# MustaphaMensouri/Distributed-Continuous-Training-with-Airflow-PyTorch-Distributed-DDP-

Measured on AMD Instinct MI355X. Metric: samples/sec (whole node) for weather-MLP DDP, higher is better.
Workload: dtype fp32; 1 GPU; global_batch=4, per_rank_batch=4, parallelism=dp1, optimizer=adam lr=0.01, loss=ce, engine=fused-persistent, dataset_rows=8649, features=5

## Files before the change

### distributed-continuous-training-with-airflow-pytorch-distributed-ddp-_amd/csrc/knobs.cpp

```cpp
#include "knobs.h"

#include <cstdlib>
#include <cstring>

namespace dct {

namespace {
Knobs g_knobs;
bool g_loaded = false;

int env_int(const char* name, int dflt) {
  const char* e = std::getenv(name);
  return (e && *e) ? std::atoi(e) : dflt;
}
}

void knobs_reload() {
  Knobs k;
  const char* mk = std::getenv("DCT_MLP_KERNEL");
  k.mlp_force_lds = (mk && std::strcmp(mk, "lds") == 0) ? 1 : 0;
  if (const char* b = std::getenv("DCT_MLP_BLOCK")) k.mlp_block = (b[0] == '0') ? 0 : (b[0] == '3' ? 3 : (b[0] == '8' ? 8 : -1));
  k.fused_head = env_int("DCT_FUSED_HEAD", 1) != 0;
  k.dw_into_adam = env_int("DCT_DW_INTO_ADAM", 1) != 0;
  k.reducer_inline = env_int("DCT_REDUCER_INLINE", -2);
  if (k.reducer_inline > 1 || k.reducer_inline < -2) k.reducer_inline = -2;
  k.rccl_one_rank = env_int("DCT_RCCL_ONE_RANK", 0) == 1;
  k.reducer_standin_us = env_int("DCT_REDUCER_STANDIN_US", 0);
  k.reducer_standin_wgs = env_int("DCT_REDUCER_STANDIN_WGS", 16);
  k.reducer_flag_edges = env_int("DCT_REDUCER_FLAG_EDGES", 1) != 0;
  if (k.reducer_standin_us < 0) k.reducer_standin_us = 0;
  if (k.reducer_standin_wgs < 1) k.reducer_standin_wgs = 1;
  if (k.reducer_standin_wgs > 1024) k.reducer_standin_wgs = 1024;
  g_knobs = k;
  g_loaded = true;
}

const Knobs& knobs() {
  if (!g_loaded) knobs_reload();
  return g_knobs;
}

}

extern "C" void dct_knobs_reload() { dct::knobs_reload(); }
```

### distributed-continuous-training-with-airflow-pytorch-distributed-ddp-_amd/csrc/knobs.h

```cpp
#pragma once

namespace dct {

struct Knobs {
  int mlp_force_lds = 0;
  int mlp_block = -1;
  int fused_head = 1;
  int dw_into_adam = 1;
  int reducer_inline = -2;
  int reducer_standin_us = 0;
  int reducer_standin_wgs = 16;
  int reducer_flag_edges = 1;
  int rccl_one_rank = 0;
};

const Knobs& knobs();
void knobs_reload();

}
```

### distributed-continuous-training-with-airflow-pytorch-distributed-ddp-_amd/csrc/mlp_block5.hip

```cpp
#include "mlp_block5_impl.h"

namespace dct {

void mlp_launch_block5_xg(int world, size_t bytes, hipStream_t st, const MlpShape& sh, const MlpArgs& a);
void mlp_launch_block5_b8(size_t bytes, hipStream_t st, const MlpShape& sh, const MlpArgs& a);

static bool b5_xg_world_ok(int w) { return w >= 2 && w <= 8; }

bool mlp_block5_ok(const MlpShape& sh, const MlpArgs& a) {
  const bool aligned = (sh.woff[1] % 4) == 0 && ((uintptr_t)a.p & 15) == 0 && (((uintptr_t)a.m | (uintptr_t)a.v) & 15) == 0;
  const bool xg_ok = a.xg_world <= 1 ||
                     (a.mode == 0 && b5_xg_world_ok(a.xg_world) && a.xg_rank >= 0 && a.xg_rank < a.xg_world &&
                      a.xg_recv != nullptr && a.xg_peers != nullptr && a.xg_status != nullptr &&
                      (a.prof == nullptr || a.xg_world == 2 || a.xg_world == 4 || a.xg_world == 8));
  const bool b8_ok = (a.B <= blk5::B && sh.mlp_block != 8) || a.prof == nullptr;
  return aligned && b8_ok && mlp_block5_shape_ok(sh.dims, sh.L, a.B) &&
         ((a.mode == 0 && a.cursor == nullptr) || (a.mode == 1 && a.steps == 1 && a.grad_out != nullptr)) &&
         (a.loss_kind == 0 || a.loss_kind == 1) && a.pending == nullptr && (a.stage == nullptr || a.mode == 1) && xg_ok;
}

bool mlp_block5_shape_ok(const int* dims, int L, int B) {
  return L == 3 && dims[1] == blk5::H && dims[2] == blk5::H && dims[0] >= 1 && dims[0] <= blk5::DMAX &&
         dims[3] == blk5::C && B >= 1 && B <= blk5::BMAX;
}

size_t mlp_block5_xg_bytes(int world) {
  switch (world) {
    case 2: return (size_t)b5x::Lay<2>::BYTES;
    case 4: return (size_t)b5x::Lay<4>::BYTES;
    case 8: return (size_t)b5x::Lay<8>::BYTES;
    case 3: return (size_t)b5x::Lay<3>::BYTES;
    case 5: return (size_t)b5x::Lay<5>::BYTES;
    case 6: return (size_t)b5x::Lay<6>::BYTES;
    case 7: return (size_t)b5x::Lay<7>::BYTES;
    default: return 0;
  }
}

hipError_t mlp_launch_block5(const MlpShape& sh, const MlpArgs& a, hipStream_t st) {
  const size_t bytes = (size_t)blk5::LDS_FLOATS * sizeof(float);
  const bool wd = a.wd != 0.f;
  if (a.B > blk5::B || sh.mlp_block == 8) {
    mlp_launch_block5_b8(bytes, st, sh, a);
  } else if (a.xg_world > 1) {
    mlp_launch_block5_xg(a.xg_world, bytes, st, sh, a);
  } else if (a.mode == 1) {
    if (a.loss_kind == 0) b5_launch<false, 0, false, true, false>(bytes, st, sh, a);
    else b5_launch<false, 1, false, true, false>(bytes, st, sh, a);
  } else if (a.prof) {
    if (a.loss_kind == 0) b5_launch<true, 0, true>(bytes, st, sh, a);
    else b5_launch<true, 1, true>(bytes, st, sh, a);
  } else if (a.loss_kind == 0) {
    if (wd) b5_launch<true, 0>(bytes, st, sh, a);
    else b5_launch<false, 0>(bytes, st, sh, a);
  } else {
    if (wd) b5_launch<true, 1>(bytes, st, sh, a);
    else b5_launch<false, 1>(bytes, st, sh, a);
  }
  return hipGetLastError();
}

}
```

### distributed-continuous-training-with-airflow-pytorch-distributed-ddp-_amd/csrc/mlp_block5_impl.h

```cpp
#pragma once
#include <type_traits>

#include "mlp_block_util.h"

namespace dct {

namespace blk5 {
constexpr int H = 128, NT = 512, NW = 8, KS = 16, DMAX = 8, B = 4, C = 2, MBMAX = 2, BMAX = B * MBMAX;
constexpr int PSTR = 36;
template <int MB>
struct Lds {
  static constexpr int RB = B * MB;
  static constexpr int XT = 0;
  static constexpr int LAB = XT + 3 * DMAX * RB;
  static constexpr int MSK = LAB + (MB == 1 ? 16 : 32);
  static constexpr int LOGP = MSK + 2 * NW * 2;
  static constexpr int H1W = LOGP + 2 * NW * 8;
  static constexpr int H1X = H1W + MB * NW * KS * 4;
  static constexpr int PART = H1X + NW * KS * 4;
  static constexpr int W2L = PART + 2 * H * PSTR;
  static constexpr int B2L = W2L + 2 * H * C;
  static constexpr int ABT = B2L + 8;
  static constexpr int TOTAL = ABT + 4;
  static_assert((H1W % 4) == 0 && (PART % 4) == 0 && (MSK % 4) == 0 && (LAB % 4) == 0 && (W2L % 4) == 0 &&
                    (B2L % 4) == 0 && (H1X % 4) == 0 && (LOGP % 4) == 0,
                "16-B aligned tiles");
};
static_assert(Lds<1>::TOTAL == 11036, "the batch <= 4 layout is round 5's");
constexpr int STG = H * H;
constexpr int LDS_FLOATS = Lds<MBMAX>::TOTAL > 2 * STG ? Lds<MBMAX>::TOTAL : 2 * STG;
static_assert(LDS_FLOATS * 4 <= 160 * 1024, "fits the CU");
using Stg = bku::Stage<H, NT>;
constexpr float LOG2E = 1.4426950408889634f, LN2 = 0.6931471805599453f;
}

namespace b5x {
typedef unsigned int v4u __attribute__((ext_vector_type(4)));
constexpr int SYS = 17;
constexpr int NP = 16, NS = 2;
constexpr int G = blk5::NT * 16;
template <int XW>
struct Lay {
  static constexpr int NO = (NP + XW - 1) / XW;
  static constexpr int RSS = NO + NS;
  static constexpr int AG = 2 * XW * RSS * G;
  static constexpr int LS = AG + 2 * (NP + NS) * G;
  static constexpr int EP = LS + ((2 * XW * 16 + 255) & ~255);
  static constexpr int BYTES = EP + (NP + NS) * 2 * G;
  static __device__ __forceinline__ int rs(int par, int src, int slot) { return ((par * XW + src) * RSS + slot) * G; }
  static __device__ __forceinline__ int ag(int par, int slot) { return AG + (par * (NP + NS) + slot) * G; }
  static __device__ __forceinline__ int ls(int par, int src) { return LS + (par * XW + src) * 16; }
  static __device__ __forceinline__ int ep(int slot, int mv) { return EP + (slot * 2 + mv) * G; }
};
__device__ __forceinline__ void put(__amdgpu_buffer_rsrc_t rs, int off, float x, float y, uint32_t tag) {
  v4u d;
  d.x = __float_as_uint(x);
  d.y = tag;
  d.z = __float_as_uint(y);
  d.w = tag;
  __builtin_amdgcn_raw_buffer_store_b128(d, rs, off, 0, SYS);
}
__device__ __forceinline__ bool get(__amdgpu_buffer_rsrc_t rs, int off, uint32_t tag, float& x, float& y) {
  const v4u d = __builtin_amdgcn_raw_buffer_load_b128(rs, off, 0, SYS);
  x = __uint_as_float(d.x);
  y = __uint_as_float(d.z);
  return (d.y == tag) & (d.w == tag);
}
template <int XW, class T>
__device__ __forceinline__ T pick(const T* v, int rank) {
  T r = v[0];
#pragma unroll
  for (int k = 1; k < XW; ++k) r = rank == k ? v[k] : r;
  return r;
}
template <int V>
using IC = std::integral_constant<int, V>;
template <int N, int I = 0, class F>
__device__ __host__ __forceinline__ void static_for(F&& f) {
  if constexpr (I < N) {
    f(IC<I>{});
    static_for<N, I + 1>(f);
  }
}
}

#define B5STAMP(k)                                              \
  if constexpr (PROF) {                                         \
    const unsigned long long t_ = __builtin_amdgcn_s_memtime(); \
    pacc[(k)] += t_ - t_last;                                   \
    t_last = t_;                                                \
  }

__device__ __forceinline__ uint32_t b5_elem(int li, int r, int u) {
  return ((uint32_t)((li * 64 + r) * 65536 + u) + 0x165667B1u) * 0xC2B2AE3Du;
}
__device__ __forceinline__ float b5_drop(uint32_t seed, uint32_t gstep, uint32_t elem, float p, float scale) {
  uint32_t h = (seed * 0x9E3779B1u) ^ ((gstep + 0x7F4A7C15u) * 0x85EBCA77u);
  h ^= elem;
  h ^= h >> 16;
  h *= 0x7feb352du;
  h ^= h >> 15;
  h *= 0x846ca68bu;
  h ^= h >> 16;
  return u01(h) < p ? 0.f : scale;
}

template <bool WD>
__device__ __forceinline__ void adam_pair(float& p0, float g0, float& m0, float& v0, float& p1, float g1, float& m1,
                                          float& v1, float b1, float b2, float wd, float A, float E) {
  if constexpr (WD) { g0 = fmaf(wd, p0, g0); g1 = fmaf(wd, p1, g1); }
  m0 = fmaf(b1, m0, g0);
  m1 = fmaf(b1, m1, g1);
  v0 = fmaf(b2, v0, g0 * g0);
  v1 = fmaf(b2, v1, g1 * g1);
  const float d0 = fmaf(__builtin_amdgcn_sqrtf(v0), A, E), d1 = fmaf(__builtin_amdgcn_sqrtf(v1), A, E);
  const float R = __builtin_amdgcn_rcpf(d0 * d1);
  p0 = fmaf(-m0, d1 * R, p0);
  p1 = fmaf(-m1, d0 * R, p1);
}

__device__ __forceinline__ bku::f32x4_t quad_transpose_mf(const float (&v)[4], const float (&e)[4]) {
  bku::f32x4_t t = (bku::f32x4_t){0.f, 0.f, 0.f, 0.f};
#pragma unroll
  for (int i = 0; i < 4; ++i) t = bku::mfma4(v[i], e[i], t);
  return t;
}

__device__ __forceinline__ float rs_bits2to5(float (&P)[16], int lane) {
  using namespace bku;
#pragma unroll
  for (int i = 0; i < 8; ++i) P[i] = swap32_sum(P[i], P[i + 8]);
#pragma unroll
  for (int i = 0; i < 4; ++i) P[i] = swap16_sum(P[i], P[i + 4]);
  const bool b3 = (lane >> 3) & 1, b2 = (lane >> 2) & 1;
#pragma unroll
  for (int i = 0; i < 2; ++i) {
    const float keep = b3 ? P[i + 2] : P[i], send = b3 ? P[i] : P[i + 2];
    P[i] = keep + dpp<ROR8>(send);
  }
  const float keep = b2 ? P[1] : P[0], send = b2 ? P[0] : P[1];
  const float t4 = dpp<ROR4>(send), t12 = dpp<0x12C>(send);
  return keep + (b2 ? t4 : t12);
}

typedef float v2f __attribute__((ext_vector_type(2)));
template <bool WD>
__device__ __forceinline__ void adam_v2(v2f& p, v2f g, v2f& m, v2f& v, float b1, float b2, float wd, float A, float E) {
  if constexpr (WD) g = (v2f)(wd) * p + g;
  m = (v2f)(b1) * m + g;
  v = (v2f)(b2) * v + g * g;
  const v2f sq = (v2f){__builtin_amdgcn_sqrtf(v.x), __builtin_amdgcn_sqrtf(v.y)};
  const v2f d = sq * (v2f)(A) + (v2f)(E);
  const float R = __builtin_amdgcn_rcpf(d.x * d.y);
  p = p - m * ((v2f){d.y, d.x} * R);
}

template <bool WD, int LK, bool PROF = false, bool DXM = true, bool ADAM = true, int XW = 1, int RK = -1, int MB = 1>
__global__ __launch_bounds__(blk5::NT, 1) void mlp_block5_kernel(MlpShape sh, MlpArgs a) {
  using namespace blk5;
  using namespace bku;
  static_assert(XW == 1 || (ADAM && XW >= 2 && XW <= 8), "exchange: train mode, 2..8 ranks");
  static_assert(MB >= 1 && MB <= MBMAX, "micro-batches per step");
  using LY = Lds<MB>;
  constexpr int RB = LY::RB, XT = LY::XT, LAB = LY::LAB, MSK = LY::MSK, LOGP = LY::LOGP, H1W = LY::H1W;
  constexpr int H1X = LY::H1X, PART = LY::PART, W2L = LY::W2L, B2L = LY::B2L, ABT = LY::ABT, TOTAL = LY::TOTAL;
  constexpr int PS = XW > 1 ? 32 : 16;
  using XL = b5x::Lay<XW>;
  constexpr int NO = XL::NO;
  extern __shared__ __attribute__((aligned(16))) float lds[];
  const int tid = threadIdx.x, w = tid >> 6, l = tid & 63;
  const int D0 = sh.dims[0];
  const int r0 = l & 3;
  const int u = KS * w + (l >> 2);
  const int wo0 = sh.woff[0], bo0 = sh.boff[0], wo1 = sh.woff[1], bo1 = sh.boff[1];
  const int wo2 = sh.woff[2], bo2 = sh.boff[2];
  unsigned long long pacc[PROF ? PS : 1] = {};
  unsigned long long t_last = PROF ? __builtin_amdgcn_s_memtime() : 0ull;
  const unsigned long long t_kstart = t_last;

  const int Bsz = a.B;
  const int fb = tid & (RB - 1), fd = tid / RB;
  const int nel = Bsz * D0;
  int role = 0, pb = 0, pk = 0;
  if (tid < nel) { role = 1; pb = tid / D0; pk = tid - pb * D0; }
  else if (tid < nel + Bsz) { role = 2; pb = tid - nel; }
  const bool stp = !ADAM && a.stage != nullptr;
  uint32_t st_tag = 0u, st_x = 0u, st_lab = 0u;
  if (stp) {
    st_tag = a.stage[0];
    if (tid < RB * DMAX && fd < D0 && fb < Bsz) st_x = a.stage[64 + fb * D0 + fd];
    if (tid < Bsz) st_lab = a.stage[64 + nel + tid];
  }
  const int cur0 = (!ADAM && a.cursor) ? sload(a.cursor) : 0;
  const int bs0 = min(Bsz, a.n_items - cur0 * Bsz);
  const bool first_ok = tid < RB * DMAX && fb < bs0;
  const int rb_raw = a.idx[max(0, min(cur0 * Bsz + (first_ok ? fb : 0), a.n_items - 1))];
  const int rb_first = (first_ok && !stp) ? rb_raw : 0;
  int ridx_next = 0;
  if (!stp && role && (cur0 + 1) * Bsz + pb < a.n_items) ridx_next = a.idx[(cur0 + 1) * Bsz + pb];

  v4f sp[Stg::LD], sm[Stg::LD], sv[Stg::LD];
#pragma unroll
  for (int i = 0; i < Stg::LD; ++i) {
    const int f = wo1 + 4 * (i * NT + tid);
    sp[i] = *reinterpret_cast<const v4f*>(a.p + f);
    if constexpr (ADAM) sm[i] = *reinterpret_cast<const v4f*>(a.m + f);
  }
  if constexpr (ADAM) {
#pragma unroll
    for (int i = 0; i < Stg::LD; ++i) sv[i] = *reinterpret_cast<const v4f*>(a.v + wo1 + 4 * (i * NT + tid));
  }
  float w0[2], m0[2], v0[2];
#pragma unroll
  for (int i = 0; i < 2; ++i) {
    const int d = r0 + 4 * i;
    const bool ok = d < D0;
    const int f = wo0 + u * D0 + (ok ? d : 0);
    w0[i] = ok ? a.p[f] : 0.f;
    m0[i] = (ok && ADAM) ? a.m[f] : 0.f;
    v0[i] = (ok && ADAM) ? a.v[f] : 0.f;
  }
  float pb0 = a.p[bo0 + u], mb0 = ADAM ? a.m[bo0 + u] : 0.f, vb0 = ADAM ? a.v[bo0 + u] : 0.f;
  float pw2[C];
#pragma unroll
  for (int c = 0; c < C; ++c) pw2[c] = a.p[wo2 + c * H + u];
  const bool own_w2 = r0 < C;
  const int fw2 = wo2 + (XW > 1 ? (r0 & 1) : (own_w2 ? r0 : 0)) * H + u;
  float mw2 = ((own_w2 || XW > 1) && ADAM) ? a.m[fw2] : 0.f, vw2 = ((own_w2 || XW > 1) && ADAM) ? a.v[fw2] : 0.f;
  float pb1 = a.p[bo1 + u], mb1 = ADAM ? a.m[bo1 + u] : 0.f, vb1 = ADAM ? a.v[bo1 + u] : 0.f;
  const bool own_b2 = w == 0 && l < C;
  const int fb2 = bo2 + (own_b2 ? l : 0);
  float pb2 = own_b2 ? a.p[fb2] : 0.f, mb2 = (own_b2 && ADAM) ? a.m[fb2] : 0.f, vb2 = (own_b2 && ADAM) ? a.v[fb2] : 0.f;
  const int fbx = r0 == 0 ? bo0 + u : (r0 == 1 ? bo1 + u : bo2 + (l & 1));
  float pbx = 0.f, mbx = 0.f, vbx = 0.f;
  if constexpr (XW > 1) {
    pbx = a.p[fbx];
    mbx = a.m[fbx];
    vbx = a.v[fbx];
  }

  int t0 = a.t0;
  uint32_t step_base = a.step_base;
  if (a.step_counter) {
    t0 = sload(a.step_counter);
    step_base = (uint32_t)t0;
// ... 47 lines not shown
  const uint32_t* pf_base = role == 1 ? reinterpret_cast<const uint32_t*>(a.X) + pk : reinterpret_cast<const uint32_t*>(a.Y);
  const int pf_stride = role == 1 ? a.ldx : (role == 2 ? 1 : 0);
  lds_barrier();

  if constexpr (PROF) pacc[14] = __builtin_amdgcn_s_memtime() - t_kstart;
  const float p_drop = a.dropout;
  const bool drop = p_drop > 0.f;
  const float scale = XW > 1 ? a.k_drop_scale : (drop ? 1.0f / (1.0f - p_drop) : 1.0f);
  const float l2b1 = XW > 1 ? a.k_l2b1 : log2f(a.b1), l2b2 = XW > 1 ? a.k_l2b2 : log2f(a.b2);
  const float c1 = 1.f - a.b1, c2 = 1.f - a.b2;
  const float rc1 = XW > 1 ? a.k_rc1 : 1.f / c1, rc2 = XW > 1 ? a.k_rc2 : 1.f / c2;
  const float sqc2 = XW > 1 ? a.k_sqc2 : sqrtf(c2);
#pragma unroll
  for (int j = 0; j < 2; ++j)
#pragma unroll
    for (int k = 0; k < KS; ++k) { m1[j][k] *= rc1; v1[j][k] *= rc2; }
#pragma unroll
  for (int i = 0; i < 2; ++i) { m0[i] *= rc1; v0[i] *= rc2; }
  mb0 *= rc1; vb0 *= rc2; mw2 *= rc1; vw2 *= rc2; mb1 *= rc1; vb1 *= rc2; mb2 *= rc1; vb2 *= rc2;
  mbx *= rc1; vbx *= rc2;
  v2f W[2][KS / 2], Mo[2][KS / 2], Vo[2][KS / 2];
#pragma unroll
  for (int j = 0; j < 2; ++j)
#pragma unroll
    for (int h = 0; h < KS / 2; ++h) {
      W[j][h] = (v2f){w1[j][2 * h], w1[j][2 * h + 1]};
      Mo[j][h] = (v2f){m1[j][2 * h], m1[j][2 * h + 1]};
      Vo[j][h] = (v2f){v1[j][2 * h], v1[j][2 * h + 1]};
    }
  const int xrank = XW > 1 ? (RK >= 0 ? RK : a.xg_rank) : 0;
  v2f MoO[NO], VoO[NO];
  __amdgpu_buffer_rsrc_t xrr = __builtin_amdgcn_make_buffer_rsrc((void*)a.xg_recv, 0, 0, 0x00020000), xpr[XW];
  const bool sown = XW == 1 || (__builtin_amdgcn_readfirstlane(w) % XW) == xrank;
  bool xbad = false;
  unsigned long long xticks = 0;
  if constexpr (XW > 1) {
#pragma unroll
    for (int t = 0; t < NO; ++t) {
      v2f cm[XW], cv[XW];
#pragma unroll
      for (int k = 0; k < XW; ++k) {
        const int i = XW * t + k < b5x::NP ? XW * t + k : 0;
        cm[k] = Mo[i >> 3][i & 7];
        cv[k] = Vo[i >> 3][i & 7];
      }
      MoO[t] = b5x::pick<XW>(cm, xrank);
      VoO[t] = b5x::pick<XW>(cv, xrank);
    }
  }
  if constexpr (XW > 1) {
    xrr = __builtin_amdgcn_make_buffer_rsrc((void*)a.xg_recv, 0, XL::BYTES, 0x00020000);
#pragma unroll
    for (int q = 0; q < XW; ++q)
      xpr[q] = __builtin_amdgcn_make_buffer_rsrc((void*)sload_ptr(a.xg_peers, q), 0, XL::BYTES, 0x00020000);
  }
  auto xwait = [&](uint32_t tag, auto&& sweep) -> bool {
    const unsigned long long t_start = __builtin_amdgcn_s_memrealtime();
    for (int spin = 0;; ++spin) {
      asm volatile("" ::: "memory");
      if (__all(sweep())) return true;
      if ((spin & 15) == 15 && (long long)(__builtin_amdgcn_s_memrealtime() - t_start) > a.xg_timeout) {
        if (l == 0) __hip_atomic_store(a.xg_status, tag, __ATOMIC_RELAXED, __HIP_MEMORY_SCOPE_SYSTEM);
        return false;
      }
      __builtin_amdgcn_s_sleep(1);
    }
  };
  const int tb = tid * 16;
  uint32_t el0[MB], el1[MB];
  float f1[MB], f2[MB];
#pragma unroll
  for (int hf = 0; hf < MB; ++hf) {
    el0[hf] = b5_elem(0, r0 + B * hf, u);
    el1[hf] = b5_elem(1, r0 + B * hf, u);
    f1[hf] = b5_drop(a.seed, step_base, el0[hf], p_drop, scale);
    f2[hf] = b5_drop(a.seed, step_base, el1[hf], p_drop, scale);
  }
  float* h1x = lds + H1X + w * (KS * 4);
  float eye[4];
#pragma unroll
  for (int i = 0; i < 4; ++i) eye[i] = r0 == i ? 1.f : 0.f;
  const int cb = (l >> 2) & 1;
  int xb = 0;
  if (a.tune == 1 && w >= NW / 2) __builtin_amdgcn_s_setprio(1);
  if (a.tune == 2 && w < NW / 2) __builtin_amdgcn_s_setprio(1);
  if constexpr (PROF) {
    t_last = __builtin_amdgcn_s_memtime();
    pacc[9] = t_last - t_kstart;
  }
  for (int s = 0; s < a.steps; ++s) {
    const int sb = s + cur0;
    const int bs = min(Bsz, a.n_items - sb * Bsz);
    const uint32_t gstep = step_base + (uint32_t)s;
    const int xbn = xb == 2 ? 0 : xb + 1;
    const int pbuf = s & 1, nbuf = pbuf ^ 1;
    const float* xT = lds + XT + xb * DMAX * RB;
    const bool have_next = (s + 1 < a.steps);
    const int bs_next = have_next ? min(Bsz, a.n_items - (sb + 1) * Bsz) : 0;
    const uint32_t raw_next = pf_base[(size_t)ridx_next * pf_stride];
    const int nx2 = min((sb + 2) * Bsz + pb, a.n_items - 1);
    const int ridx_next2 = a.idx[nx2 < 0 ? 0 : nx2];
    const uint32_t xtag = gstep + 1u;
    const int xpar = (int)(gstep & 1u);
    const int t = t0 + s + 1;
    float dz2m[MB][2][4];
    float dz = 0.f, xbl = 0.f, tls = 0.f;
    float h2 = 0.f, h1 = 0.f;
    float gw0s = 0.f, gw1s = 0.f, gb1s = 0.f, gbs = 0.f, g0s = 0.f, g1s = 0.f, db0s = 0.f;
    float aA = 0.f, aE = 0.f;
    v2f GO[NO];
#pragma unroll
    for (int t2 = 0; t2 < NO; ++t2) GO[t2] = (v2f){0.f, 0.f};
    float xg_own = 0.f, xg_bx = 0.f;
    v2f xs_g0 = (v2f){0.f, 0.f}, xs_g1 = (v2f){0.f, 0.f};
    bool abort_step = false;
    auto dw1_pass = [&]() {
#pragma unroll
      for (int q = 0; q < KS / 4; ++q) {
        f32x4_t g[2];
#pragma unroll
        for (int j = 0; j < 2; ++j) g[j] = (f32x4_t){0.f, 0.f, 0.f, 0.f};
#pragma unroll
        for (int hf = 0; hf < MB; ++hf) {
          const float4 hq = *reinterpret_cast<const float4*>(lds + H1W + (hf * NW + w) * (KS * 4) + (4 * q + r0) * 4);
          const float hv[4] = {hq.x, hq.y, hq.z, hq.w};
#pragma unroll
          for (int j = 0; j < 2; ++j)
#pragma unroll
            for (int r = 0; r < 4; ++r) g[j] = mfma4(hv[r], dz2m[hf][j][r], g[j]);
        }

        if constexpr (ADAM && XW > 1) {
#pragma unroll
          for (int j = 0; j < 2; ++j)
#pragma unroll
            for (int h = 0; h < 2; ++h) {
              const int i = 8 * j + 2 * q + h;
              const float gx = g[j][2 * h], gy = g[j][2 * h + 1];
              if ((i % XW) == xrank) GO[i / XW] = (v2f){gx, gy};
              else b5x::put(xpr[i % XW], XL::rs(xpar, (xrank - i % XW + XW) % XW, i / XW) + tb, gx, gy, xtag);
            }
        } else if constexpr (ADAM) {
#pragma unroll
          for (int j = 0; j < 2; ++j)
#pragma unroll
            for (int h = 0; h < 2; ++h)
              adam_v2<WD>(W[j][2 * q + h], (v2f){g[j][2 * h], g[j][2 * h + 1]}, Mo[j][2 * q + h], Vo[j][2 * q + h], a.b1,
                          a.b2, a.wd, aA, aE);
        } else {
#pragma unroll
          for (int j = 0; j < 2; ++j)
            *reinterpret_cast<float4*>(a.grad_out + wo1 + (l + 64 * j) * H + KS * w + 4 * q) =
                make_float4(g[j][0], g[j][1], g[j][2], g[j][3]);
        }
      }
    };

#pragma unroll
    for (int hf = 0; hf < MB; ++hf) {
      const bool last = hf == MB - 1;
      const int mpar = MB == 1 ? pbuf : hf;
      float* h1w = lds + H1W + (hf * NW + w) * (KS * 4);

      const float4 xa = *reinterpret_cast<const float4*>(xT + r0 * RB + B * hf);
      const float4 xc = *reinterpret_cast<const float4*>(xT + (r0 + 4) * RB + B * hf);
      {
        const float acc0 = w0[0] * xa.x + w0[1] * xc.x, acc1 = w0[0] * xa.y + w0[1] * xc.y;
        const float acc2 = w0[0] * xa.z + w0[1] * xc.z, acc3 = w0[0] * xa.w + w0[1] * xc.w;
        const bool qb1 = (r0 >> 1) & 1, qb0 = r0 & 1;
        const float k0 = qb1 ? acc2 : acc0, k1 = qb1 ? acc3 : acc1;
        const float s0 = qb1 ? acc0 : acc2, s1 = qb1 ? acc1 : acc3;
        const float e0 = k0 + dpp<QP_X2>(s0), e1 = k1 + dpp<QP_X2>(s1);
        const float kq = qb0 ? e1 : e0, sq = qb0 ? e0 : e1;
        h1 = fmaxf(kq + dpp<QP_X1>(sq) + pb0, 0.f) * f1[hf];
        h1w[l] = h1;
        h1x[r0 * KS + (l >> 2)] = h1;
      }
      __builtin_amdgcn_wave_barrier();
      B5STAMP(0)
      {
        f32x4_t cq[2][KS / 4];
#pragma unroll
        for (int q = 0; q < KS / 4; ++q) {
          const float4 hq = *reinterpret_cast<const float4*>(h1x + r0 * KS + 4 * q);
          const float hv[4] = {hq.x, hq.y, hq.z, hq.w};
#pragma unroll
          for (int j = 0; j < 2; ++j) {
            cq[j][q] = (f32x4_t){0.f, 0.f, 0.f, 0.f};
#pragma unroll
            for (int e = 0; e < 4; ++e) cq[j][q] = mfma4(hv[e], W[j][2 * q + (e >> 1)][e & 1], cq[j][q]);
          }
        }
        f32x4_t cj[2];
#pragma unroll
        for (int j = 0; j < 2; ++j) cj[j] = (cq[j][0] + cq[j][1]) + (cq[j][2] + cq[j][3]);
        float* part = lds + PART + mpar * (H * PSTR);
#pragma unroll
        for (int j = 0; j < 2; ++j)
          *reinterpret_cast<float4*>(part + (l + 64 * j) * PSTR + w * 4) = make_float4(cj[j][0], cj[j][1], cj[j][2], cj[j][3]);
      }
      if (hf == 0) {
        if (stp) {
          const int bs_st = min(Bsz, a.n_items - (sb + 1) * Bsz);
          if (role) a.stage[64 + tid] = pb < bs_st ? raw_next : 0u;
          if (tid == 0) a.stage[0] = bs_st > 0 ? (uint32_t)(sb + 2) : 0u;
        }
        if (role) {
          const uint32_t v = (have_next && pb < bs_next) ? raw_next : 0u;
          uint32_t* dst = (role == 1) ? reinterpret_cast<uint32_t*>(lds + XT + xbn * DMAX * RB) + pk * RB + pb
                                      : reinterpret_cast<uint32_t*>(lds + LAB) + xbn * RB + pb;
          *dst = v;
        }
        ridx_next = role ? ridx_next2 : 0;
      }
      B5STAMP(1)
      lds_barrier();
      B5STAMP(2)
      if constexpr (XW > 1) {
        if (lds[ABT] != 0.f) {
          abort_step = true;
          break;
        }
      }

      const float2 wv0 = *reinterpret_cast<const float2*>(lds + W2L + pbuf * (H * C) + l * C);
      const float2 wv1 = *reinterpret_cast<const float2*>(lds + W2L + pbuf * (H * C) + (l + 64) * C);
      const float b2c = lds[B2L + pbuf * 4 + cb];
      const int lab = reinterpret_cast<const int*>(lds + LAB)[xb * RB + B * hf + r0];
      {
        const float* pr = lds + PART + mpar * (H * PSTR) + u * PSTR + r0;
        float q[NW];
#pragma unroll
        for (int ww = 0; ww < NW; ++ww) q[ww] = pr[4 * ww];
        const float z = ((q[0] + q[1]) + (q[2] + q[3])) + ((q[4] + q[5]) + (q[6] + q[7]));
        h2 = fmaxf(z + pb1, 0.f) * f2[hf];
        const float t0s = sum_bits2to5(pw2[0] * h2), t1s = sum_bits2to5(pw2[1] * h2);
        const unsigned long long msk = __ballot(h2 > 0.f);
        if (l < 8) lds[LOGP + mpar * (NW * 8) + w * 8 + l] = cb ? t1s : t0s;
        if (l == 0)
          *reinterpret_cast<uint2*>(lds + MSK + mpar * (NW * 2) + w * 2) = make_uint2((uint32_t)msk, (uint32_t)(msk >> 32));
      }
      B5STAMP(3)
      lds_barrier();
      B5STAMP(4)

      const uint2 mw0 = *reinterpret_cast<const uint2*>(lds + MSK + mpar * (NW * 2) + 2 * (l >> 4));
      const uint2 mw1 = *reinterpret_cast<const uint2*>(lds + MSK + mpar * (NW * 2) + 2 * ((l >> 4) + 4));
      float lv;
      {
        float lg = lds[LOGP + mpar * (NW * 8) + l];
        lg += dpp<ROR8>(lg);
        lg = swap16_sum(lg, lg);
        lg = swap32_sum(lg, lg);
        const float z = lg + b2c;
        const float zo = dpp<ROR4>(z);
        const bool live = r0 + B * hf < bs;
        const float invb = __builtin_amdgcn_rcpf((float)(bs > 0 ? bs : 1));
        const float inv = live ? invb : 0.f;
        const float y = (cb == lab) ? 1.f : 0.f;
        if constexpr (LK == 0) {
          const float tt = zo - z;
          const float e = __builtin_amdgcn_exp2f(tt * LOG2E);
          const float pc = __builtin_amdgcn_rcpf(1.f + e);
          dz = (pc - y) * inv;
          const float sp = fmaxf(tt, 0.f) + LN2 * __builtin_amdgcn_logf(1.f + __builtin_amdgcn_exp2f(-fabsf(tt) * LOG2E));
          lv = (live && cb == lab) ? sp : 0.f;
        } else {
          const float d = z - y;
          dz = d * inv;
          lv = live ? 0.5f * d * d : 0.f;
        }
      }
      float dz3[4][C];
#pragma unroll
      for (int r = 0; r < 4; ++r)
#pragma unroll
        for (int c = 0; c < C; ++c) dz3[r][c] = rl(dz, 4 * c + r);
      if (w == 0) {
        float tl = lv + dpp<QP_X1>(lv);
        tl += dpp<QP_X2>(tl);
        tl += dpp<ROR4>(tl);
        tls = hf == 0 ? tl : tls + tl;
        if (last) {
          const float bl = bs > 0 ? tls * __builtin_amdgcn_rcpf((float)bs) : 0.f;
          if constexpr (ADAM && XW > 1) {
            xbl = rl(bl, 0);
            if (l == 0) {
#pragma unroll
              for (int q = 0; q < XW; ++q)
                if (q != xrank) b5x::put(xpr[q], XL::ls(xpar, xrank), xbl, 0.f, xtag);
            }
          } else if constexpr (ADAM) {
            if (l == 0 && a.loss_out) a.loss_out[s] = bl;
          } else {
            if (l == 0) a.grad_out[sh.P] = bl;
          }
        }
      }
      B5STAMP(5)

      if (last) {
        const float step_size = a.lr * __builtin_amdgcn_rcpf(1.f - pow_t(l2b1, (float)t));
        const float rbc2 = __builtin_amdgcn_rsqf(1.f - pow_t(l2b2, (float)t));
        const float rss = __builtin_amdgcn_rcpf(step_size);
        aA = sqc2 * rbc2 * rss * rc1;
        aE = a.eps * rss * rc1;
      }
      {
        const int sh4 = 4 * (l & 15);
#pragma unroll
        for (int j = 0; j < 2; ++j) {
          const float2 wv = j ? wv1 : wv0;
          const uint2 mw = j ? mw1 : mw0;
          const uint32_t nib = ((sh4 < 32 ? mw.x : mw.y) >> (sh4 & 31)) & 15u;
#pragma unroll
          for (int r = 0; r < 4; ++r) {
            const float g = wv.x * dz3[r][0] + wv.y * dz3[r][1];
            dz2m[hf][j][r] = ((nib >> r) & 1u) ? g * scale : 0.f;
          }
        }
      }
      if constexpr (XW > 1) {
        if (last) {
          dw1_pass();
          B5STAMP(15)
        }
      }
      {
        const float d_own = dz, d_oth = dpp<ROR4>(dz);
        const float dr0 = cb ? d_oth : d_own, dr1 = cb ? d_own : d_oth;
        const float gw0 = quad_sum(dr0 * h2), gw1 = quad_sum(dr1 * h2);
        float gdz = pw2[0] * dr0 + pw2[1] * dr1;
        gdz = h2 > 0.f ? gdz * scale : 0.f;
        const float gb1 = quad_sum(gdz);
        const float gbh = (l & 1) ? (dz3[0][1] + dz3[1][1]) + (dz3[2][1] + dz3[3][1])
                                  : (dz3[0][0] + dz3[1][0]) + (dz3[2][0] + dz3[3][0]);
        gw0s = hf == 0 ? gw0 : gw0s + gw0;
        gw1s = hf == 0 ? gw1 : gw1s + gw1;
        gb1s = hf == 0 ? gb1 : gb1s + gb1;
        gbs = hf == 0 ? gbh : gbs + gbh;
        if (last) {
          float pown = (r0 & 1) ? pw2[1] : pw2[0];
          const float gown = (r0 & 1) ? gw1s : gw0s;
          const float gb = gbs;
          if constexpr (ADAM && XW > 1) {
            xg_own = gown;
            xg_bx = r0 == 1 ? gb1s : gb;
          } else if constexpr (ADAM) {
            adam_pair<WD>(pown, gown, mw2, vw2, pb1, gb1s, mb1, vb1, a.b1, a.b2, a.wd, aA, aE);
            pw2[0] = dpp<QB0>(pown);
            pw2[1] = dpp<QB1>(pown);
            if (own_w2) lds[W2L + nbuf * (H * C) + u * C + r0] = pown;
            adam_scaled<WD>(pb2, gb, mb2, vb2, a.b1, a.b2, a.wd, aA, aE);
            if (own_b2) lds[B2L + nbuf * 4 + l] = pb2;
          } else {
            if (own_w2) a.grad_out[fw2] = gown;
            if (r0 == 0) a.grad_out[bo1 + u] = gb1s;
            if (own_b2) a.grad_out[fb2] = gb;
          }
        }
      }
      B5STAMP(6)
      float dz1 = 0.f;
      if constexpr (DXM) {
        float dzt[2][4];
#pragma unroll
        for (int j = 0; j < 2; ++j) {
          const f32x4_t tq = quad_transpose_mf(dz2m[hf][j], eye);
#pragma unroll
          for (int i = 0; i < 4; ++i) dzt[j][i] = tq[i];
        }
        float P[16];
#pragma unroll
        for (int q = 0; q < KS / 4; ++q) {
          f32x4_t acc[2];
#pragma unroll
          for (int j = 0; j < 2; ++j) {
            const float wq[4] = {W[j][2 * q].x, W[j][2 * q].y, W[j][2 * q + 1].x, W[j][2 * q + 1].y};
            const f32x4_t wt = quad_transpose_mf(wq, eye);
            acc[j] = (f32x4_t){0.f, 0.f, 0.f, 0.f};
#pragma unroll
            for (int i = 0; i < 4; ++i) acc[j] = mfma4(wt[i], dzt[j][i], acc[j]);
          }
          const f32x4_t at = acc[0] + acc[1];
#pragma unroll
          for (int m = 0; m < 4; ++m) P[4 * q + m] = at[m];
        }
        dz1 = rs_bits2to5(P, l);
      } else {
#pragma unroll
        for (int p = 0; p < 4; ++p) {
          float P[16];
#pragma unroll
          for (int kk = 0; kk < KS; ++kk)
            P[kk] = W[0][kk >> 1][kk & 1] * dz2m[hf][0][p] + W[1][kk >> 1][kk & 1] * dz2m[hf][1][p];
          const float tot = rs_small<16>(P, l);
          if (r0 == p) dz1 = tot;
        }
      }
      dz1 = h1 > 0.f ? dz1 * scale : 0.f;
      {
        const float dq0 = dpp<QB0>(dz1), dq1 = dpp<QB1>(dz1), dq2 = dpp<QB2>(dz1), dq3 = dpp<QB3>(dz1);
        const float g0h = dq0 * xa.x + dq1 * xa.y + dq2 * xa.z + dq3 * xa.w;
        const float g1h = dq0 * xc.x + dq1 * xc.y + dq2 * xc.z + dq3 * xc.w;
        const float dbh = (dq0 + dq1) + (dq2 + dq3);
        g0s = hf == 0 ? g0h : g0s + g0h;
        g1s = hf == 0 ? g1h : g1s + g1h;
        db0s = hf == 0 ? dbh : db0s + dbh;
        if (last) {
          const float g0 = g0s, g1 = g1s;
          if constexpr (ADAM && XW > 1) {
            if (r0 == 0) xg_bx = db0s;
            xs_g0 = (v2f){g0, g1};
            xs_g1 = (v2f){xg_own, xg_bx};
            if (!sown) {
#pragma unroll
              for (int q = 0; q < XW; ++q)
                if (q == __builtin_amdgcn_readfirstlane(w) % XW) {
                  const int rel = (xrank - q + XW) % XW;
                  b5x::put(xpr[q], XL::rs(xpar, rel, NO) + tb, g0, g1, xtag);
                  b5x::put(xpr[q], XL::rs(xpar, rel, NO + 1) + tb, xg_own, xg_bx, xtag);
                }
            }
          } else if constexpr (ADAM) {
            adam_pair<WD>(w0[0], g0, m0[0], v0[0], w0[1], g1, m0[1], v0[1], a.b1, a.b2, a.wd, aA, aE);
            adam_scaled<WD>(pb0, db0s, mb0, vb0, a.b1, a.b2, a.wd, aA, aE);
          } else {
            if (r0 < D0) a.grad_out[wo0 + u * D0 + r0] = g0;
            if (r0 + 4 < D0) a.grad_out[wo0 + u * D0 + r0 + 4] = g1;
            if (r0 == 0) a.grad_out[bo0 + u] = db0s;
          }
        }
      }
    }
    if constexpr (XW > 1) {
      if (abort_step) break;
    }
#pragma unroll
    for (int hf = 0; hf < MB; ++hf) {
      f1[hf] = b5_drop(a.seed, gstep + 1u, el0[hf], p_drop, scale);
      f2[hf] = b5_drop(a.seed, gstep + 1u, el1[hf], p_drop, scale);
    }
    B5STAMP(7)
    if constexpr (XW == 1) dw1_pass();
    if constexpr (ADAM && XW > 1) {
      const unsigned long long xt0 = __builtin_amdgcn_s_memrealtime();
      const float invw = 1.f / (float)XW;
      do {
        float rv[XW][NO][2], sv[XW][2][2];
        if (!xwait(xtag, [&]() -> bool {
              bool k = true;
#pragma unroll
              for (int q = 1; q < XW; ++q)
#pragma unroll
                for (int t = 0; t < NO; ++t)
                  k &= b5x::get(xrr, XL::rs(xpar, q, t) + tb, xtag, rv[q][t][0], rv[q][t][1]) | (XW * t + xrank >= b5x::NP);
              return k;
            })) {
          xbad = true;
          break;
        }
        B5STAMP(16)
        auto small_sweep = [&]() -> bool {
          bool k = true;
#pragma unroll
          for (int q = 1; q < XW; ++q) {
            k &= b5x::get(xrr, XL::rs(xpar, q, NO) + tb, xtag, sv[q][0][0], sv[q][0][1]);
            k &= b5x::get(xrr, XL::rs(xpar, q, NO + 1) + tb, xtag, sv[q][1][0], sv[q][1][1]);
          }
          return k;
        };
        bool sok = true;
        if (sown) sok = small_sweep();
        v2f WO[NO];
#pragma unroll
        for (int t = 0; t < NO; ++t) {
          v2f cw[XW];
#pragma unroll
          for (int k = 0; k < XW; ++k) {
            const int i = XW * t + k < b5x::NP ? XW * t + k : 0;
            cw[k] = W[i >> 3][i & 7];
          }
          WO[t] = b5x::pick<XW>(cw, xrank);
          v2f gs = GO[t];
#pragma unroll
          for (int q = 1; q < XW; ++q) gs += (v2f){rv[q][t][0], rv[q][t][1]};
          adam_v2<WD>(WO[t], gs * (v2f)(invw), MoO[t], VoO[t], a.b1, a.b2, a.wd, aA, aE);
          const int agoff = XL::ag(xpar, XW * t + xrank) + tb;
          if (XW * t + xrank < b5x::NP) {
#pragma unroll
            for (int q = 0; q < XW; ++q)
              if (q != xrank) b5x::put(xpr[q], agoff, WO[t].x, WO[t].y, xtag);
          }
        }
        B5STAMP(17)
        if (sown && !__all(sok) && !xwait(xtag, small_sweep)) {
          xbad = true;
          break;
        }
        if (sown) {
          v2f s0 = xs_g0, s1 = xs_g1;
#pragma unroll
          for (int q = 1; q < XW; ++q) {
            s0 += (v2f){sv[q][0][0], sv[q][0][1]};
            s1 += (v2f){sv[q][1][0], sv[q][1][1]};
          }
          s0 *= (v2f)(invw);
          s1 *= (v2f)(invw);
          adam_pair<WD>(w0[0], s0.x, m0[0], v0[0], w0[1], s0.y, m0[1], v0[1], a.b1, a.b2, a.wd, aA, aE);
          float pown = (r0 & 1) ? pw2[1] : pw2[0];
          adam_pair<WD>(pown, s1.x, mw2, vw2, pbx, s1.y, mbx, vbx, a.b1, a.b2, a.wd, aA, aE);
          xs_g1.x = pown;
#pragma unroll
          for (int q = 0; q < XW; ++q)
            if (q != xrank) {
              b5x::put(xpr[q], XL::ag(xpar, b5x::NP) + tb, w0[0], w0[1], xtag);
              b5x::put(xpr[q], XL::ag(xpar, b5x::NP + 1) + tb, pown, pbx, xtag);
            }
        }
        B5STAMP(18)
        float av[b5x::NP][2], sa[2][2], lq = 0.f, lq1;
        const int lsrc = l < XW ? l : 0;
        const bool lskip = w != 0 || l >= XW || l == xrank;
        if (!xwait(xtag, [&]() -> bool {
// ... 109 lines not shown
      }
    } while (false);
    if (xbad) lds[ABT] = 1.f;
    lds_barrier();
    if (lds[ABT] != 0.f) return;
    mbx *= c1;
    vbx *= c2;
  }
  if (a.step_counter && tid == 0)
    __hip_atomic_store(a.step_counter, t0 + a.steps, __ATOMIC_RELAXED, __HIP_MEMORY_SCOPE_AGENT);
  if constexpr (!ADAM) {
    if (a.cursor && tid == 0) __hip_atomic_store(a.cursor, cur0 + a.steps, __ATOMIC_RELAXED, __HIP_MEMORY_SCOPE_AGENT);
    return;
  }

  int lo = l, uo = u, to = tid;
  asm volatile("" : "+v"(lo), "+v"(uo), "+v"(to));
#pragma unroll
  for (int j = 0; j < 2; ++j)
#pragma unroll
    for (int h = 0; h < KS / 2; ++h) {
      w1[j][2 * h] = W[j][h].x; w1[j][2 * h + 1] = W[j][h].y;
      m1[j][2 * h] = Mo[j][h].x; m1[j][2 * h + 1] = Mo[j][h].y;
      v1[j][2 * h] = Vo[j][h].x; v1[j][2 * h + 1] = Vo[j][h].y;
    }
#pragma unroll
  for (int j = 0; j < 2; ++j)
#pragma unroll
    for (int k = 0; k < KS; ++k) { m1[j][k] *= c1; v1[j][k] *= c2; }
#pragma unroll
  for (int i = 0; i < 2; ++i) { m0[i] *= c1; v0[i] *= c2; }
  mb0 *= c1; vb0 *= c2; mw2 *= c1; vw2 *= c2; mb1 *= c1; vb1 *= c2; mb2 *= c1; vb2 *= c2;
  lds_barrier();
  Stg::own<KS>(lds, w1, lo, KS / 4 * w);
  Stg::own<KS>(lds + STG, m1, lo, KS / 4 * w);
  lds_barrier();
  Stg::store(a.p + wo1, lds, to);
  Stg::store(a.m + wo1, lds + STG, to);
  lds_barrier();
  Stg::own<KS>(lds, v1, lo, KS / 4 * w);
  lds_barrier();
  Stg::store(a.v + wo1, lds, to);
  const int r0o = lo & 3;
#pragma unroll
  for (int i = 0; i < 2; ++i) {
    const int d = r0o + 4 * i;
    if (d < D0) {
      const int f = wo0 + uo * D0 + d;
      a.p[f] = w0[i];
      a.m[f] = m0[i];
      a.v[f] = v0[i];
    }
  }
  if constexpr (XW > 1) {
    if (r0o < 2 || (w == 0 && (lo == 2 || lo == 3))) {
      a.p[fbx] = pbx; a.m[fbx] = mbx; a.v[fbx] = vbx;
    }
    if (own_w2) {
      const int f = wo2 + r0o * H + uo;
      a.p[f] = (r0o & 1) ? pw2[1] : pw2[0]; a.m[f] = mw2; a.v[f] = vw2;
    }
  } else {
    if (r0o == 0) {
      a.p[bo0 + uo] = pb0; a.m[bo0 + uo] = mb0; a.v[bo0 + uo] = vb0;
      a.p[bo1 + uo] = pb1; a.m[bo1 + uo] = mb1; a.v[bo1 + uo] = vb1;
    }
    if (own_w2) {
      const int f = wo2 + r0o * H + uo;
      a.p[f] = (r0o & 1) ? pw2[1] : pw2[0]; a.m[f] = mw2; a.v[f] = vw2;
    }
    if (own_b2) { a.p[fb2] = pb2; a.m[fb2] = mb2; a.v[fb2] = vb2; }
  }
  if constexpr (PROF) {
    asm volatile("s_waitcnt vmcnt(0)" ::: "memory");
    pacc[10] = __builtin_amdgcn_s_memtime() - t_last;
    if (l == 0) {
#pragma unroll
      for (int i = 0; i < PS - 1; ++i) atomicAdd(a.prof + w * PS + i, pacc[i]);
    }
  }
}
#undef B5STAMP

template <bool WD, int LK, bool PROF = false, bool DXM = true, bool ADAM = true, int XW = 1, int RK = -1, int MB = 1>
inline void b5_launch(size_t bytes, hipStream_t st, const MlpShape& sh, const MlpArgs& a) {
  static const hipError_t attr = hipFuncSetAttribute((const void*)mlp_block5_kernel<WD, LK, PROF, DXM, ADAM, XW, RK, MB>,
                                                     hipFuncAttributeMaxDynamicSharedMemorySize, (int)bytes);
  (void)attr;
  hipLaunchKernelGGL((mlp_block5_kernel<WD, LK, PROF, DXM, ADAM, XW, RK, MB>), dim3(1), dim3(blk5::NT), bytes, st, sh, a);
}


}
```

Baseline: 1.046 million samples/s.

## Schedule dropout, Adam scalars and weight transposes into a latency gap in block5 kernel

Adds a compile-time step-schedule mask to the single-rank block5 training kernel and makes it the default. Three pieces of independent work move into a wait window after the hidden-layer partial-sum read: next-step dropout masks, a per-64-step lane table of Adam bias-correction scalars, and the first backward weight quad-transposes. The aim is to hide latency on the serial per-step critical path. The cost is extra live registers, and an env knob plus A/B variants allow falling back.

```diff
diff --git a/distributed-continuous-training-with-airflow-pytorch-distributed-ddp-_amd/csrc/knobs.cpp b/distributed-continuous-training-with-airflow-pytorch-distributed-ddp-_amd/csrc/knobs.cpp
--- a/distributed-continuous-training-with-airflow-pytorch-distributed-ddp-_amd/csrc/knobs.cpp
+++ b/distributed-continuous-training-with-airflow-pytorch-distributed-ddp-_amd/csrc/knobs.cpp
@@ -20,6 +20,8 @@
   const char* mk = std::getenv("DCT_MLP_KERNEL");
   k.mlp_force_lds = (mk && std::strcmp(mk, "lds") == 0) ? 1 : 0;
   if (const char* b = std::getenv("DCT_MLP_BLOCK")) k.mlp_block = (b[0] == '0') ? 0 : (b[0] == '3' ? 3 : (b[0] == '8' ? 8 : -1));
+  k.b5_sched = env_int("DCT_B5_SCHED", -1);
+  if (k.b5_sched < 0) k.b5_sched = -1;
   k.fused_head = env_int("DCT_FUSED_HEAD", 1) != 0;
   k.dw_into_adam = env_int("DCT_DW_INTO_ADAM", 1) != 0;
   k.reducer_inline = env_int("DCT_REDUCER_INLINE", -2);
diff --git a/distributed-continuous-training-with-airflow-pytorch-distributed-ddp-_amd/csrc/knobs.h b/distributed-continuous-training-with-airflow-pytorch-distributed-ddp-_amd/csrc/knobs.h
--- a/distributed-continuous-training-with-airflow-pytorch-distributed-ddp-_amd/csrc/knobs.h
+++ b/distributed-continuous-training-with-airflow-pytorch-distributed-ddp-_amd/csrc/knobs.h
@@ -5,6 +5,7 @@
 struct Knobs {
   int mlp_force_lds = 0;
   int mlp_block = -1;
+  int b5_sched = -1;
   int fused_head = 1;
   int dw_into_adam = 1;
   int reducer_inline = -2;
diff --git a/distributed-continuous-training-with-airflow-pytorch-distributed-ddp-_amd/csrc/mlp_block5.hip b/distributed-continuous-training-with-airflow-pytorch-distributed-ddp-_amd/csrc/mlp_block5.hip
--- a/distributed-continuous-training-with-airflow-pytorch-distributed-ddp-_amd/csrc/mlp_block5.hip
+++ b/distributed-continuous-training-with-airflow-pytorch-distributed-ddp-_amd/csrc/mlp_block5.hip
@@ -1,3 +1,4 @@
+#include "knobs.h"
 #include "mlp_block5_impl.h"
 
 namespace dct {
@@ -37,9 +38,34 @@
   }
 }
 
+template <bool WD, int LK, bool PROF = false>
+static void b5_launch_sched(int sched, size_t bytes, hipStream_t st, const MlpShape& sh, const MlpArgs& a) {
+  using namespace blk5;
+  if (sched == 0) return b5_launch<WD, LK, PROF>(bytes, st, sh, a);
+#ifdef B5_SCHED_AB
+  if constexpr (!WD && LK == 0 && !PROF) {
+    constexpr int D = SCHED_DEFAULT;
+    constexpr int NWT = D & ~(SCH_WT1 | SCH_WT2);
+    constexpr int masks[] = {SCH_DROP, SCH_ADAM_TAB, SCH_WT1, SCH_WT2, SCH_WT1 | SCH_WT2, NWT, NWT | SCH_WT2,
+                             NWT | SCH_WT1 | SCH_WT2, D & ~SCH_DROP, D & ~SCH_ADAM_TAB};
+    bool done = false;
+    b5x::static_for<sizeof(masks) / sizeof(masks[0])>([&](auto i) {
+      constexpr int M = masks[decltype(i)::value];
+      if (!done && sched == 256 + M && M != D) {
+        b5_launch<WD, LK, false, true, true, 1, -1, 1, M>(bytes, st, sh, a);
+        done = true;
+      }
+    });
+    if (done) return;
+  }
+#endif
+  b5_launch<WD, LK, PROF, true, true, 1, -1, 1, SCHED_DEFAULT>(bytes, st, sh, a);
+}
+
 hipError_t mlp_launch_block5(const MlpShape& sh, const MlpArgs& a, hipStream_t st) {
   const size_t bytes = (size_t)blk5::LDS_FLOATS * sizeof(float);
   const bool wd = a.wd != 0.f;
+  const int sched = knobs().b5_sched;
   if (a.B > blk5::B || sh.mlp_block == 8) {
     mlp_launch_block5_b8(bytes, st, sh, a);
   } else if (a.xg_world > 1) {
@@ -48,14 +74,14 @@
     if (a.loss_kind == 0) b5_launch<false, 0, false, true, false>(bytes, st, sh, a);
     else b5_launch<false, 1, false, true, false>(bytes, st, sh, a);
   } else if (a.prof) {
-    if (a.loss_kind == 0) b5_launch<true, 0, true>(bytes, st, sh, a);
-    else b5_launch<true, 1, true>(bytes, st, sh, a);
+    if (a.loss_kind == 0) b5_launch_sched<true, 0, true>(sched, bytes, st, sh, a);
+    else b5_launch_sched<true, 1, true>(sched, bytes, st, sh, a);
   } else if (a.loss_kind == 0) {
-    if (wd) b5_launch<true, 0>(bytes, st, sh, a);
-    else b5_launch<false, 0>(bytes, st, sh, a);
+    if (wd) b5_launch_sched<true, 0>(sched, bytes, st, sh, a);
+    else b5_launch_sched<false, 0>(sched, bytes, st, sh, a);
   } else {
-    if (wd) b5_launch<true, 1>(bytes, st, sh, a);
-    else b5_launch<false, 1>(bytes, st, sh, a);
+    if (wd) b5_launch_sched<true, 1>(sched, bytes, st, sh, a);
+    else b5_launch_sched<false, 1>(sched, bytes, st, sh, a);
   }
   return hipGetLastError();
 }
diff --git a/distributed-continuous-training-with-airflow-pytorch-distributed-ddp-_amd/csrc/mlp_block5_impl.h b/distributed-continuous-training-with-airflow-pytorch-distributed-ddp-_amd/csrc/mlp_block5_impl.h
--- a/distributed-continuous-training-with-airflow-pytorch-distributed-ddp-_amd/csrc/mlp_block5_impl.h
+++ b/distributed-continuous-training-with-airflow-pytorch-distributed-ddp-_amd/csrc/mlp_block5_impl.h
@@ -32,6 +32,8 @@
 static_assert(LDS_FLOATS * 4 <= 160 * 1024, "fits the CU");
 using Stg = bku::Stage<H, NT>;
 constexpr float LOG2E = 1.4426950408889634f, LN2 = 0.6931471805599453f;
+constexpr int SCH_DROP = 1, SCH_ADAM_TAB = 2, SCH_WT1 = 8, SCH_WT2 = 16;
+constexpr int SCHED_DEFAULT = SCH_DROP | SCH_ADAM_TAB | SCH_WT1;
 }
 
 namespace b5x {
@@ -155,12 +157,16 @@
   p = p - m * ((v2f){d.y, d.x} * R);
 }
 
-template <bool WD, int LK, bool PROF = false, bool DXM = true, bool ADAM = true, int XW = 1, int RK = -1, int MB = 1>
+template <bool WD, int LK, bool PROF = false, bool DXM = true, bool ADAM = true, int XW = 1, int RK = -1, int MB = 1,
+          int SCH = 0>
 __global__ __launch_bounds__(blk5::NT, 1) void mlp_block5_kernel(MlpShape sh, MlpArgs a) {
   using namespace blk5;
   using namespace bku;
   static_assert(XW == 1 || (ADAM && XW >= 2 && XW <= 8), "exchange: train mode, 2..8 ranks");
   static_assert(MB >= 1 && MB <= MBMAX, "micro-batches per step");
+  static_assert(SCH == 0 || (XW == 1 && MB == 1 && ADAM), "step-schedule items: one-rank train mode, one micro-batch");
+  constexpr bool S_DROP = (SCH & SCH_DROP) != 0, S_TAB = (SCH & SCH_ADAM_TAB) != 0;
+  constexpr int HQ = DXM ? (SCH / SCH_WT1) & 3 : 0;
   using LY = Lds<MB>;
   constexpr int RB = LY::RB, XT = LY::XT, LAB = LY::LAB, MSK = LY::MSK, LOGP = LY::LOGP, H1W = LY::H1W;
   constexpr int H1X = LY::H1X, PART = LY::PART, W2L = LY::W2L, B2L = LY::B2L, ABT = LY::ABT, TOTAL = LY::TOTAL;
@@ -374,6 +380,7 @@
   for (int i = 0; i < 4; ++i) eye[i] = r0 == i ? 1.f : 0.f;
   const int cb = (l >> 2) & 1;
   int xb = 0;
+  float tabA = 0.f, tabE = 0.f;
   if (a.tune == 1 && w >= NW / 2) __builtin_amdgcn_s_setprio(1);
   if (a.tune == 2 && w < NW / 2) __builtin_amdgcn_s_setprio(1);
   if constexpr (PROF) {
@@ -400,6 +407,8 @@
     float h2 = 0.f, h1 = 0.f;
     float gw0s = 0.f, gw1s = 0.f, gb1s = 0.f, gbs = 0.f, g0s = 0.f, g1s = 0.f, db0s = 0.f;
     float aA = 0.f, aE = 0.f;
+    float f1n = 0.f, f2n = 0.f;
+    f32x4_t wth[HQ > 0 ? HQ : 1][2];
     v2f GO[NO];
 #pragma unroll
     for (int t2 = 0; t2 < NO; ++t2) GO[t2] = (v2f){0.f, 0.f};
@@ -524,6 +533,40 @@
         float q[NW];
 #pragma unroll
         for (int ww = 0; ww < NW; ++ww) q[ww] = pr[4 * ww];
+        if constexpr (SCH != 0) {
+          __builtin_amdgcn_sched_barrier(0);
+          if constexpr (HQ > 0) {
+#pragma unroll
+            for (int qq = 0; qq < HQ; ++qq)
+#pragma unroll
+              for (int j = 0; j < 2; ++j) {
+                const float wq[4] = {W[j][2 * qq].x, W[j][2 * qq].y, W[j][2 * qq + 1].x, W[j][2 * qq + 1].y};
+                wth[qq][j] = quad_transpose_mf(wq, eye);
+              }
+          }
+          if constexpr (S_DROP) {
+            uint32_t gnext = gstep + 1u;
+            asm volatile("" : "+s"(gnext));
+            f1n = b5_drop(a.seed, gnext, el0[0], p_drop, scale);
+            f2n = b5_drop(a.seed, gnext, el1[0], p_drop, scale);
+            asm volatile("" : "+v"(f1n), "+v"(f2n));
+          }
+          if constexpr (S_TAB) {
+            const int ti = s & 63;
+            if (ti == 0) {
+              asm volatile("");
+              const float tl = (float)(t + l);
+              const float step_size = a.lr * __builtin_amdgcn_rcpf(1.f - pow_t(l2b1, tl));
+              const float rbc2 = __builtin_amdgcn_rsqf(1.f - pow_t(l2b2, tl));
+              const float rss = __builtin_amdgcn_rcpf(step_size);
+              tabA = sqc2 * rbc2 * rss * rc1;
+              tabE = a.eps * rss * rc1;
+            }
+            aA = rl(tabA, ti);
+            aE = rl(tabE, ti);
+          }
+          __builtin_amdgcn_sched_barrier(0);
+        }
         const float z = ((q[0] + q[1]) + (q[2] + q[3])) + ((q[4] + q[5]) + (q[6] + q[7]));
         h2 = fmaxf(z + pb1, 0.f) * f2[hf];
         const float t0s = sum_bits2to5(pw2[0] * h2), t1s = sum_bits2to5(pw2[1] * h2);
@@ -591,7 +634,7 @@
       }
       B5STAMP(5)
 
-      if (last) {
+      if (last && !S_TAB) {
         const float step_size = a.lr * __builtin_amdgcn_rcpf(1.f - pow_t(l2b1, (float)t));
         const float rbc2 = __builtin_amdgcn_rsqf(1.f - pow_t(l2b2, (float)t));
         const float rss = __builtin_amdgcn_rcpf(step_size);
@@ -669,7 +712,7 @@
 #pragma unroll
           for (int j = 0; j < 2; ++j) {
             const float wq[4] = {W[j][2 * q].x, W[j][2 * q].y, W[j][2 * q + 1].x, W[j][2 * q + 1].y};
-            const f32x4_t wt = quad_transpose_mf(wq, eye);
+            const f32x4_t wt = q < HQ ? wth[q < HQ ? q : 0][j] : quad_transpose_mf(wq, eye);
             acc[j] = (f32x4_t){0.f, 0.f, 0.f, 0.f};
 #pragma unroll
             for (int i = 0; i < 4; ++i) acc[j] = mfma4(wt[i], dzt[j][i], acc[j]);
@@ -728,10 +771,15 @@
     if constexpr (XW > 1) {
       if (abort_step) break;
     }
-#pragma unroll
-    for (int hf = 0; hf < MB; ++hf) {
-      f1[hf] = b5_drop(a.seed, gstep + 1u, el0[hf], p_drop, scale);
-      f2[hf] = b5_drop(a.seed, gstep + 1u, el1[hf], p_drop, scale);
+    if constexpr (S_DROP) {
+      f1[0] = f1n;
+      f2[0] = f2n;
+    } else {
+#pragma unroll
+      for (int hf = 0; hf < MB; ++hf) {
+        f1[hf] = b5_drop(a.seed, gstep + 1u, el0[hf], p_drop, scale);
+        f2[hf] = b5_drop(a.seed, gstep + 1u, el1[hf], p_drop, scale);
+      }
     }
     B5STAMP(7)
     if constexpr (XW == 1) dw1_pass();
@@ -1007,13 +1055,14 @@
 }
 #undef B5STAMP
 
-template <bool WD, int LK, bool PROF = false, bool DXM = true, bool ADAM = true, int XW = 1, int RK = -1, int MB = 1>
+template <bool WD, int LK, bool PROF = false, bool DXM = true, bool ADAM = true, int XW = 1, int RK = -1, int MB = 1,
+          int SCH = 0>
 inline void b5_launch(size_t bytes, hipStream_t st, const MlpShape& sh, const MlpArgs& a) {
-  static const hipError_t attr = hipFuncSetAttribute((const void*)mlp_block5_kernel<WD, LK, PROF, DXM, ADAM, XW, RK, MB>,
+  static const hipError_t attr = hipFuncSetAttribute((const void*)mlp_block5_kernel<WD, LK, PROF, DXM, ADAM, XW, RK, MB, SCH>,
                                                      hipFuncAttributeMaxDynamicSharedMemorySize, (int)bytes);
   (void)attr;
-  hipLaunchKernelGGL((mlp_block5_kernel<WD, LK, PROF, DXM, ADAM, XW, RK, MB>), dim3(1), dim3(blk5::NT), bytes, st, sh, a);
-}
-
-
-}
+  hipLaunchKernelGGL((mlp_block5_kernel<WD, LK, PROF, DXM, ADAM, XW, RK, MB, SCH>), dim3(1), dim3(blk5::NT), bytes, st, sh, a);
+}
+
+
+}
```

Result: faster. 1.092 million samples/s (median of 6 runs) (+4.4%).
